# crowsonkb/k-diffusion

Measured on NVIDIA H100. Metric: images/sec (256x256, Heun 50-step), higher is better.
Workload: dtype bf16

## Files before the change

k-diffusion_b200/csrc/tc_kernels.cu:

```cuda
#include "tc_common.cuh"
#include "tc_kernels.cuh"

namespace kdb {

typedef CUresult (*EncodeTiledFn)(CUtensorMap*, CUtensorMapDataType, cuuint32_t, void*, const cuuint64_t*, const cuuint64_t*,
                                  const cuuint32_t*, const cuuint32_t*, CUtensorMapInterleave, CUtensorMapSwizzle,
                                  CUtensorMapL2promotion, CUtensorMapFloatOOBfill);

static EncodeTiledFn encode_fn() {
  static EncodeTiledFn fn = [] {
    void* p = nullptr;
    cudaDriverEntryPointQueryResult q;
    if (cudaGetDriverEntryPoint("cuTensorMapEncodeTiled", &p, cudaEnableDefault, &q) != cudaSuccess) p = nullptr;
    return reinterpret_cast<EncodeTiledFn>(p);
  }();
  return fn;
}

int make_tmap_bf16(CUtensorMap* out, const void* base, int rank, const uint64_t* dims, const uint64_t* strides_bytes, const uint32_t* box) {
  EncodeTiledFn fn = encode_fn();
  KDB_REQUIRE(fn != nullptr, KDB_ERR_UNSUPPORTED, "cuTensorMapEncodeTiled not available from this driver");
  cuuint64_t gd[5];
  cuuint64_t gs[5];
  cuuint32_t bx[5], es[5];
  for (int i = 0; i < rank; ++i) {
    gd[i] = dims[i];
    bx[i] = box[i];
    es[i] = 1;
    if (i > 0) gs[i - 1] = strides_bytes[i - 1];
  }
  CUresult r = fn(out, CU_TENSOR_MAP_DATA_TYPE_BFLOAT16, (cuuint32_t)rank, const_cast<void*>(base), gd, gs, bx, es,
                  CU_TENSOR_MAP_INTERLEAVE_NONE, CU_TENSOR_MAP_SWIZZLE_128B, CU_TENSOR_MAP_L2_PROMOTION_L2_256B,
                  CU_TENSOR_MAP_FLOAT_OOB_FILL_NONE);
  KDB_REQUIRE(r == CUDA_SUCCESS, KDB_ERR_BAD_ARG, "cuTensorMapEncodeTiled failed with CUresult %d (rank %d, dim0 %llu, box0 %u)", (int)r,
              rank, (unsigned long long)dims[0], box[0]);
  return 0;
}

int make_tmap_tokens(CUtensorMap* out, const void* base, uint64_t C, int B, int h, int w, uint32_t box_c, uint32_t box_w, uint32_t box_h) {
  const uint64_t dims[4] = {C, (uint64_t)w, (uint64_t)h, (uint64_t)B};
  const uint64_t strides[3] = {C * 2, C * 2 * w, C * 2 * w * h};
  const uint32_t box[4] = {box_c, box_w, box_h, 1};
  return make_tmap_bf16(out, base, 4, dims, strides, box);
}

bool pdl_enabled() {
  static const bool enabled = [] {
    const char* e = getenv("KDB200_NO_PDL");
    return !(e != nullptr && e[0] == '1');
  }();
  return enabled;
}

namespace {

constexpr int BM = 128, BK = 64;
constexpr int A_STAGE_BYTES = BM * BK * 2;
constexpr int SUB_TILE_BYTES = BM * 128;
constexpr int GEMM_THREADS = 384;

struct GemmArgs : GemmEpi {
  bf16* out;
  int64_t M;
  int N, K;
  int box_w, box_h;
  int th, tw;
};

__device__ __forceinline__ float bf16_round(float v) { return __bfloat162float(__float2bfloat16_rn(v)); }

int tmap_2d(CUtensorMap* t, const void* base, uint64_t inner, uint64_t outer, uint32_t box_inner, uint32_t box_outer) {
  const uint64_t dims[2] = {inner, outer};
  const uint64_t strides[1] = {inner * 2};
  const uint32_t box[2] = {box_inner, box_outer};
  return make_tmap_bf16(t, base, 2, dims, strides, box);
}

int tmap_quad(CUtensorMap* t, const void* base, int C, int wc, uint64_t bhc, int box_w, int box_h) {
  const uint64_t dims[5] = {(uint64_t)C, 2, (uint64_t)wc, 2, bhc};
  const uint64_t strides[4] = {(uint64_t)C * 2, (uint64_t)C * 4, (uint64_t)wc * C * 4, (uint64_t)wc * C * 8};
  const uint32_t box[5] = {64, 1, (uint32_t)box_w, 1, (uint32_t)box_h};
  return make_tmap_bf16(t, base, 5, dims, strides, box);
}

bool quad_box(int wc, int* box_w, int* box_h) {
  if (wc >= BM) {
    if (wc % BM != 0) return false;
    *box_w = BM;
    *box_h = 1;
    return true;
  }
  if (BM % wc != 0) return false;
  *box_w = wc;
  *box_h = BM / wc;
  return true;
}

struct QuadCoord {
  int e, nw, wx, nh, row;
};
__device__ __forceinline__ QuadCoord quad_coord(int64_t m0, int n, int C, int wc, int box_h) {
  const int qd = n / C;
  return QuadCoord{n - qd * C, qd & 1, box_h == 1 ? (int)(m0 % wc) : 0, qd >> 1, (int)(m0 / wc)};
}

template <int BN, int EPI> constexpr int out_bytes() {
  return EPI == EPI_GEGLU ? SUB_TILE_BYTES : EPI == EPI_PATCH_OUT ? 0 : (BN / 64) * SUB_TILE_BYTES;
}
template <int BN, int EPI> constexpr int acc_bytes() { return EPI == EPI_GEGLU ? 0 : BM * BN * 4; }
template <int EPI> constexpr int ring_bytes() { return EPI == EPI_GEGLU ? 192 * 1024 : 96 * 1024; }
template <int BN, int EPI> constexpr size_t gemm_smem() { return 1024 + ring_bytes<EPI>() + acc_bytes<BN, EPI>() + 2 * out_bytes<BN, EPI>() + 128; }

template <int BN> __device__ __forceinline__ int stage_off(int row, int chunk) { return row * BN + ((chunk ^ (row & 7)) << 2); }
template <int BN>
__device__ __forceinline__ void stage_store(float* s, int row0, const float (&d)[BN / 2]) {
  const int t = threadIdx.x & 127;
  const int r = row0 + 16 * (t >> 5) + ((t & 31) >> 2), c = 2 * (t & 3);
#pragma unroll
  for (int j = 0; j < BN / 8; ++j) {
    *reinterpret_cast<float2*>(s + stage_off<BN>(r, 2 * j + (c >> 2)) + (c & 3)) = make_float2(d[4 * j], d[4 * j + 1]);
    *reinterpret_cast<float2*>(s + stage_off<BN>(r + 8, 2 * j + (c >> 2)) + (c & 3)) = make_float2(d[4 * j + 2], d[4 * j + 3]);
  }
}
template <int BN>
__device__ __forceinline__ void stage_ld32(const float* s, int row, int col0, float (&v)[32]) {
#pragma unroll
  for (int i = 0; i < 8; ++i) {
    const float4 q = *reinterpret_cast<const float4*>(s + stage_off<BN>(row, (col0 >> 2) + i));
    v[4 * i] = q.x;
    v[4 * i + 1] = q.y;
    v[4 * i + 2] = q.z;
    v[4 * i + 3] = q.w;
  }
}

template <int BN, int EPI>
__global__ void __launch_bounds__(GEMM_THREADS, 1) gemm_wg_kernel(const __grid_constant__ CUtensorMap tma, const __grid_constant__ CUtensorMap tmb,
                                                                  const __grid_constant__ CUtensorMap tmc, const __grid_constant__ CUtensorMap tmr,
                                                                  const GemmArgs p) {
  KDB_PDL_TRIGGER();
  constexpr int B_STAGE_BYTES = BN * BK * 2;
  constexpr int STAGE_BYTES = A_STAGE_BYTES + B_STAGE_BYTES;
  constexpr int RING_BYTES = ring_bytes<EPI>();
  constexpr int STAGES = RING_BYTES / STAGE_BYTES;
  constexpr int NSUB = BN / 64;
  constexpr bool RES = EPI == EPI_RESID;
  uint8_t* base = tc::smem_1k();
  float* sAcc = reinterpret_cast<float*>(base + RING_BYTES);
  auto* ring = reinterpret_cast<tc::TmaRing<STAGES>*>(base + RING_BYTES + acc_bytes<BN, EPI>() + 2 * out_bytes<BN, EPI>());
  uint64_t* resid_full = reinterpret_cast<uint64_t*>(ring + 1);

  const int warp = threadIdx.x >> 5, lane = threadIdx.x & 31;
  const int nkb = p.K / BK;
  const int n_tiles = p.N / BN;
  const int n_local = tc::tiles_owned((int)((p.M + BM - 1) / BM) * n_tiles);

  if (threadIdx.x == 0) {
    tc::tma_prefetch_desc(&tma);
    tc::tma_prefetch_desc(&tmb);
    ring->init(tc::REL_WARPS);
    tc::mbar_init(&resid_full[0], 1);
    tc::mbar_init(&resid_full[1], 1);
    tc::fence_barrier_init();
  }
  __syncthreads();
  tc::pdl_wait();

  if (warp >= 8) {
    tc::setmaxnreg_dec<tc::PRODUCER_REGS>();
    if (warp == 8 && tc::elect_one()) {
      int it = 0;
      for (int i = 0; i < n_local; ++i) {
        const int t = (int)blockIdx.x + i * (int)gridDim.x;
        const int64_t m0 = (int64_t)(t / n_tiles) * BM;
        const int n0 = (t % n_tiles) * BN;
        for (int kb = 0; kb < nkb; ++kb, ++it) {
          const auto ps = PipeState<STAGES>::at(it);
          uint64_t* bar = ring->acquire(ps, STAGE_BYTES);
          uint8_t* a = base + (size_t)ps.slot * STAGE_BYTES;
          if (p.mC > 0) {
            const QuadCoord q = quad_coord(m0, kb * BK, p.mC, p.mwc, p.box_h);
            tc::tma_load_5d(a, &tma, bar, q.e, q.nw, q.wx, q.nh, q.row);
          } else {
            tc::tma_load_2d(a, &tma, bar, kb * BK, (int)m0);
          }
          tc::tma_load_2d(a + A_STAGE_BYTES, &tmb, bar, kb * BK, n0);
        }
      }
    }
    return;
  }
  tc::setmaxnreg_inc<tc::MMA_REGS>();

  const int wg = warp >> 2;
  const int row = threadIdx.x & 127;
  uint8_t* sC = base + RING_BYTES + acc_bytes<BN, EPI>() + wg * out_bytes<BN, EPI>();
  const int r0 = 16 * (warp & 3) + (lane >> 2), cq = 2 * (lane & 3);
  for (int i = wg; i < n_local; i += 2) {
    const int t = (int)blockIdx.x + i * (int)gridDim.x;
    const int64_t m0 = (int64_t)(t / n_tiles) * BM;
    const int n0 = (t % n_tiles) * BN;
    if constexpr (RES || EPI == EPI_SPLIT_LERP) {
      if (row == 0 && (RES || p.box_w > 0)) {
        tc::mbar_arrive_expect_tx(&resid_full[wg], NSUB * SUB_TILE_BYTES);
#pragma unroll
        for (int g = 0; g < NSUB; ++g) {
          if constexpr (RES) {
            tc::tma_load_2d(sC + g * SUB_TILE_BYTES, &tmr, &resid_full[wg], n0 + g * 64, (int)m0);
          } else {
            const QuadCoord q = quad_coord(m0, n0 + g * 64, p.C, p.wc, p.box_h);
            tc::tma_load_5d(sC + g * SUB_TILE_BYTES, &tmr, &resid_full[wg], q.e, q.nw, q.wx, q.nh, q.row);
          }
        }
      }
    }
    float frag_rstd[4] = {1.f, 1.f, 1.f, 1.f};
    if constexpr (EPI == EPI_GEGLU) {
      if (p.ss_in != nullptr) {
#pragma unroll
        for (int h = 0; h < 4; ++h) {
          const int64_t m = m0 + r0 + 64 * (h >> 1) + 8 * (h & 1);
          const float4* sp = reinterpret_cast<const float4*>(p.ss_in + (m < p.M ? m : 0) * SS_PARTS);
          frag_rstd[h] = rsqrtf(tc::rowss_sum(__ldg(sp), __ldg(sp + 1), p.K >> 7) / (float)p.K + 1e-6f);
        }
      }
    }

    float acc0[BN / 2], acc1[BN / 2];
#pragma unroll
    for (int k = 0; k < BN / 2; ++k) acc0[k] = acc1[k] = 0.f;
    if (i > 0) tc::named_barrier_sync(tc::BAR_TURN + wg, 256);
    const int it0 = i * nkb;
    for (int kb = 0; kb < nkb; ++kb) {
      const auto ps = PipeState<STAGES>::at(it0 + kb);
      ring->wait(ps);
      const uint32_t a_addr = tc::smem_u32(base + (size_t)ps.slot * STAGE_BYTES);
      const uint64_t ad0 = tc::smem_desc_k_sw128(a_addr), ad1 = tc::smem_desc_k_sw128(a_addr + 8 * 1024);
      const uint64_t bd = tc::smem_desc_k_sw128(a_addr + A_STAGE_BYTES);
      tc::wg_fence_acc(acc0);
      tc::wg_fence_acc(acc1);
      tc::wg_fence();
#pragma unroll
      for (int k = 0; k < BK / 16; ++k) {
        if constexpr (BN == 128) {
          tc::wgmma_128(acc0, ad0 + 2ull * k, bd + 2ull * k, 1u);
          tc::wgmma_128(acc1, ad1 + 2ull * k, bd + 2ull * k, 1u);
        } else {
          tc::wgmma_64<0>(acc0, ad0 + 2ull * k, bd + 2ull * k, 1u);
          tc::wgmma_64<0>(acc1, ad1 + 2ull * k, bd + 2ull * k, 1u);
        }
      }
      tc::wg_commit();
      tc::wg_wait<1>();
      tc::wg_fence_acc(acc0);
      tc::wg_fence_acc(acc1);
      if (kb > 0 && lane == 0) ring->release(PipeState<STAGES>::at(it0 + kb - 1));
    }
    if (i + 1 < n_local) tc::named_barrier_arrive(tc::BAR_TURN + (wg ^ 1), 256);
    tc::wg_wait<0>();
    tc::wg_fence_acc(acc0);
    tc::wg_fence_acc(acc1);
    if (lane == 0) ring->release(PipeState<STAGES>::at(it0 + nkb - 1));

    if constexpr (EPI == EPI_GEGLU) {
      tc::named_barrier_sync(tc::BAR_WG + wg, 128);
#pragma unroll
      for (int half = 0; half < 2; ++half) {
        const float r_a = frag_rstd[2 * half], r_b = frag_rstd[2 * half + 1];
        uint32_t o[16];
        tc::geglu_fragment(half == 0 ? acc0 : acc1, tc::pk2(0.5f * r_a, 0.5f * r_a), tc::pk2(0.5f * r_b, 0.5f * r_b), tc::pk2(r_a, r_a),
                           tc::pk2(r_b, r_b), o);
        const int r = 64 * half + r0;
#pragma unroll
        for (int q = 0; q < 8; ++q) {
          *reinterpret_cast<uint32_t*>(sC + tc::sw128_offset(r, q) + 2 * cq) = o[2 * q];
          *reinterpret_cast<uint32_t*>(sC + tc::sw128_offset(r + 8, q) + 2 * cq) = o[2 * q + 1];
        }
      }
      tc::fence_proxy_async();
      tc::named_barrier_sync(tc::BAR_WG + wg, 128);
      if (row == 0) {
        tc::tma_store_2d(&tmc, sC, n0 / 2, (int)m0);
        tc::tma_store_commit();
        tc::tma_store_wait_read();
      }
      continue;
    }
    if (i > 0) tc::named_barrier_sync(tc::BAR_ACC + wg, 256);
    stage_store<BN>(sAcc, 0, acc0);
    stage_store<BN>(sAcc, 64, acc1);
    tc::named_barrier_sync(tc::BAR_WG + wg, 128);
    const bool pass_acc = i + 1 < n_local;

    const int64_t m = m0 + row;
    float rstd = 1.f;
    if (p.ss_in != nullptr) {
      const float4* sp = reinterpret_cast<const float4*>(p.ss_in + (m < p.M ? m : 0) * SS_PARTS);
      rstd = rsqrtf(tc::rowss_sum(__ldg(sp), __ldg(sp + 1), p.K >> 7) / (float)p.K + 1e-6f);
    }
    if constexpr (EPI == EPI_PATCH_OUT) {
      float v[64];
      {
        float t0[32], t1[32];
        stage_ld32<BN>(sAcc, row, 0, t0);
        stage_ld32<BN>(sAcc, row, 32, t1);
#pragma unroll
        for (int k = 0; k < 32; ++k) { v[k] = t0[k]; v[32 + k] = t1[k]; }
      }
      if (pass_acc) tc::named_barrier_arrive(tc::BAR_ACC + (wg ^ 1), 256);
      if (m < p.M) {
        if (p.ss_in != nullptr) {
#pragma unroll
          for (int k = 0; k < 48; ++k) v[k] *= rstd;
        }
        const int per = p.th * p.tw;
        const int b = (int)(m / per);
        const int r = (int)(m - (int64_t)b * per);
        const int ty = r / p.tw, tx = r - ty * p.tw;
        float c_skip = 0.f, c_out = 1.f, c_in;
        if (p.sigma_data > 0.f) karras_scalings(__ldg(p.sigma + b), p.sigma_data, c_skip, c_out, c_in);
#pragma unroll
        for (int c = 0; c < 3; ++c)
#pragma unroll
          for (int nh = 0; nh < 4; ++nh) {
            const int64_t o = (((int64_t)b * 3 + c) * p.H + (ty * 4 + nh)) * p.W + tx * 4;
            float4 y = make_float4(bf16_round(v[(nh * 4 + 0) * 3 + c]), bf16_round(v[(nh * 4 + 1) * 3 + c]), bf16_round(v[(nh * 4 + 2) * 3 + c]),
                                   bf16_round(v[(nh * 4 + 3) * 3 + c]));
            if (p.sigma_data > 0.f) {
              const float4 xi = __ldg(reinterpret_cast<const float4*>(p.x_in + o));
              y = make_float4(y.x * c_out + xi.x * c_skip, y.y * c_out + xi.y * c_skip, y.z * c_out + xi.z * c_skip, y.w * c_out + xi.w * c_skip);
            }
            *reinterpret_cast<float4*>(p.img + o) = y;
          }
      }
    } else if constexpr (EPI == EPI_SPLIT_LERP) {
      const bool live = m < p.M;
      const float facv = __ldg(p.fac);
      float ss = 0.f;
      int64_t fine = 0;
      if (p.box_w > 0) {
        tc::mbar_wait_nocall(&resid_full[wg], (uint32_t)(i >> 1) & 1u);
#pragma unroll 1
        for (int g = 0; g < NSUB; ++g) {
          float v[64];
          {
            float t0[32], t1[32];
            stage_ld32<BN>(sAcc, row, g * 64, t0);
            stage_ld32<BN>(sAcc, row, g * 64 + 32, t1);
#pragma unroll
            for (int k = 0; k < 32; ++k) { v[k] = t0[k]; v[32 + k] = t1[k]; }
          }
          if (g == NSUB - 1 && pass_acc) tc::named_barrier_arrive(tc::BAR_ACC + (wg ^ 1), 256);
          uint8_t* cg = sC + g * SUB_TILE_BYTES;
#pragma unroll
          for (int j = 0; j < 8; ++j) {
            uint4* cp = reinterpret_cast<uint4*>(cg + tc::sw128_offset(row, j));
            const uint4 r4 = *cp;
            const uint32_t rw[4] = {r4.x, r4.y, r4.z, r4.w};
            uint32_t ow[4];
#pragma unroll
            for (int q = 0; q < 4; ++q) {
              const float lo = __uint_as_float(rw[q] << 16), hi = __uint_as_float(rw[q] & 0xffff0000u);
              const float e0 = v[j * 8 + q * 2], e1 = v[j * 8 + q * 2 + 1];
              const float d0 = e0 - lo, d1 = e1 - hi;
              const float o0 = (facv < 0.5f) ? fmaf(facv, d0, lo) : e0 - d0 * (1.f - facv);
              const float o1 = (facv < 0.5f) ? fmaf(facv, d1, hi) : e1 - d1 * (1.f - facv);
              ss = fmaf(o0, o0, fmaf(o1, o1, ss));
              ow[q] = tc::pack_bf16x2(o0, o1);
            }
            *cp = make_uint4(ow[0], ow[1], ow[2], ow[3]);
          }
        }
        if (p.ss_out != nullptr && live) {
          const int64_t b = m / ((int64_t)p.hc * p.wc);
          const int r = (int)(m - b * p.hc * p.wc);
          const int hy = r / p.wc, wx = r - hy * p.wc, qd = n0 / p.C;
          fine = (b * (2 * p.hc) + (2 * hy + (qd >> 1))) * (2 * p.wc) + (2 * wx + (qd & 1));
          p.ss_out[fine * SS_PARTS + ((n0 % p.C) >> 7)] = ss;
        }
        tc::fence_proxy_async();
        tc::named_barrier_sync(tc::BAR_WG + wg, 128);
        if (row == 0) {
#pragma unroll
          for (int g = 0; g < NSUB; ++g) {
            const QuadCoord q = quad_coord(m0, n0 + g * 64, p.C, p.wc, p.box_h);
            tc::tma_store_5d(&tmc, sC + g * SUB_TILE_BYTES, q.e, q.nw, q.wx, q.nh, q.row);
          }
          tc::tma_store_commit();
          tc::tma_store_wait_read();
        }
        continue;
      }
#pragma unroll 1
      for (int c = 0; c < BN / 32; ++c) {
        float v[32];
        stage_ld32<BN>(sAcc, row, c * 32, v);
        if (c == BN / 32 - 1 && pass_acc) tc::named_barrier_arrive(tc::BAR_ACC + (wg ^ 1), 256);
        if (!live) continue;
        const int n = n0 + c * 32;
        const int64_t b = m / ((int64_t)p.hc * p.wc);
        const int r = (int)(m - b * p.hc * p.wc);
        const int hy = r / p.wc, wx = r - hy * p.wc;
        const int qd = n / p.C, e = n - qd * p.C;
        fine = (b * (2 * p.hc) + (2 * hy + (qd >> 1))) * (2 * p.wc) + (2 * wx + (qd & 1));
        const int64_t off = fine * p.C + e;
        const uint4* sk = reinterpret_cast<const uint4*>(static_cast<const bf16*>(p.resid) + off);
        uint4* dst = reinterpret_cast<uint4*>(p.out + off);
#pragma unroll
        for (int j = 0; j < 4; ++j) {
          const uint4 r4 = sk[j];
          const uint32_t rw[4] = {r4.x, r4.y, r4.z, r4.w};
          uint32_t ow[4];
#pragma unroll
          for (int q = 0; q < 4; ++q) {
            const float lo = __uint_as_float(rw[q] << 16), hi = __uint_as_float(rw[q] & 0xffff0000u);
            const float e0 = v[j * 8 + q * 2], e1 = v[j * 8 + q * 2 + 1];
            const float d0 = e0 - lo, d1 = e1 - hi;
            const float o0 = (facv < 0.5f) ? fmaf(facv, d0, lo) : e0 - d0 * (1.f - facv);
            const float o1 = (facv < 0.5f) ? fmaf(facv, d1, hi) : e1 - d1 * (1.f - facv);
            ss = fmaf(o0, o0, fmaf(o1, o1, ss));
            ow[q] = tc::pack_bf16x2(o0, o1);
          }
          dst[j] = make_uint4(ow[0], ow[1], ow[2], ow[3]);
        }
      }
      if (p.ss_out != nullptr && live) p.ss_out[fine * SS_PARTS + ((n0 % p.C) >> 7)] = ss;
    } else {
      if constexpr (RES) tc::mbar_wait_nocall(&resid_full[wg], (uint32_t)(i >> 1) & 1u);
      float ss_acc[4] = {0.f, 0.f, 0.f, 0.f};
#pragma unroll 1
      for (int g = 0; g < NSUB; ++g) {
        float v[64];
        {
          float t0[32], t1[32];
          stage_ld32<BN>(sAcc, row, g * 64, t0);
          stage_ld32<BN>(sAcc, row, g * 64 + 32, t1);
#pragma unroll
          for (int k = 0; k < 32; ++k) { v[k] = t0[k]; v[32 + k] = t1[k]; }
        }
        if (g == NSUB - 1 && pass_acc) tc::named_barrier_arrive(tc::BAR_ACC + (wg ^ 1), 256);
        if (p.ss_in != nullptr) {
          bool apply = true;
          if constexpr (EPI == EPI_QKV_ROPE) apply = (n0 + g * 64) >= 2 * p.C;
          if (apply) {
#pragma unroll
            for (int k = 0; k < 64; ++k) v[k] *= rstd;
          }
        }
        uint8_t* cg = sC + g * SUB_TILE_BYTES;
        if constexpr (RES) {
#pragma unroll
          for (int j = 0; j < 8; ++j) {
            const uint4 r4 = *reinterpret_cast<const uint4*>(cg + tc::sw128_offset(row, j));
            const uint32_t rw[4] = {r4.x, r4.y, r4.z, r4.w};
#pragma unroll
            for (int q = 0; q < 4; ++q) {
              v[j * 8 + q * 2] += __uint_as_float(rw[q] << 16);
              v[j * 8 + q * 2 + 1] += __uint_as_float(rw[q] & 0xffff0000u);
            }
          }
        }
        if constexpr (RES || EPI == EPI_STORE) {
          if (p.ss_out != nullptr) {
#pragma unroll
            for (int k = 0; k < 64; k += 4) {
              ss_acc[0] = fmaf(v[k], v[k], ss_acc[0]);
              ss_acc[1] = fmaf(v[k + 1], v[k + 1], ss_acc[1]);
              ss_acc[2] = fmaf(v[k + 2], v[k + 2], ss_acc[2]);
              ss_acc[3] = fmaf(v[k + 3], v[k + 3], ss_acc[3]);
            }
          }
        }
        if constexpr (EPI == EPI_QKV_ROPE) {
          const int n = n0 + g * 64;
          const int t3 = n / p.C, head = (n - t3 * p.C) >> 6;
          if (t3 < 2) {
            const int64_t tok = (m < p.M ? m : 0) % p.T_tokens;
            const float4* tb = reinterpret_cast<const float4*>(p.rope) + (int64_t)head * 8 * p.T_tokens + tok;
            tc::f32x2 P[32];
#pragma unroll
            for (int k = 0; k < 32; ++k) P[k] = tc::pk2(v[2 * k], v[2 * k + 1]);
            tc::f32x2 q0 = tc::mul2(P[0], P[0]), q1 = tc::mul2(P[1], P[1]), q2 = tc::mul2(P[2], P[2]), q3 = tc::mul2(P[3], P[3]);
#pragma unroll
            for (int k = 4; k < 32; k += 4) {
              q0 = tc::fma2(P[k], P[k], q0);
              q1 = tc::fma2(P[k + 1], P[k + 1], q1);
              q2 = tc::fma2(P[k + 2], P[k + 2], q2);
              q3 = tc::fma2(P[k + 3], P[k + 3], q3);
            }
            const float sc = sqrtf(__ldg(p.qk_scale + head)) * rsqrtf(((q0.x + q0.y) + (q1.x + q1.y)) + ((q2.x + q2.y) + (q3.x + q3.y)) + 1e-6f);
            const tc::f32x2 sc2 = tc::pk2(sc, sc);
#pragma unroll
            for (int k = 0; k < 8; ++k) {
              const float4 cs = __ldg(tb + (int64_t)k * p.T_tokens);
              const tc::f32x2 C = tc::pk2(cs.x, cs.y), S = tc::pk2(cs.z, cs.w);
              const tc::f32x2 X1 = P[k], X2 = P[8 + k];
              P[k] = tc::mul2(tc::fma2(X2, tc::neg2(S), tc::mul2(X1, C)), sc2);
              P[8 + k] = tc::mul2(tc::fma2(X1, S, tc::mul2(X2, C)), sc2);
            }
#pragma unroll
            for (int k = 16; k < 32; ++k) P[k] = tc::mul2(P[k], sc2);
#pragma unroll
            for (int k = 0; k < 32; ++k) tc::upk2(P[k], v[2 * k], v[2 * k + 1]);
          }
        }
#pragma unroll
        for (int j = 0; j < 8; ++j)
          *reinterpret_cast<uint4*>(cg + tc::sw128_offset(row, j)) =
              make_uint4(tc::pack_bf16x2(v[j * 8 + 0], v[j * 8 + 1]), tc::pack_bf16x2(v[j * 8 + 2], v[j * 8 + 3]),
                         tc::pack_bf16x2(v[j * 8 + 4], v[j * 8 + 5]), tc::pack_bf16x2(v[j * 8 + 6], v[j * 8 + 7]));
      }
      if constexpr (RES || EPI == EPI_STORE) {
        if (p.ss_out != nullptr && m < p.M) p.ss_out[m * SS_PARTS + (n0 >> 7)] = (ss_acc[0] + ss_acc[1]) + (ss_acc[2] + ss_acc[3]);
      }
      tc::fence_proxy_async();
      tc::named_barrier_sync(tc::BAR_WG + wg, 128);
      if (row == 0) {
#pragma unroll
        for (int g = 0; g < NSUB; ++g) tc::tma_store_2d(&tmc, sC + g * SUB_TILE_BYTES, n0 + g * 64, (int)m0);
        tc::tma_store_commit();
        tc::tma_store_wait_read();
      }
    }
  }
}


#include "tc_ffn_fused.cuh"
#include "tc_attn_block.cuh"

template <int BN, int EPI>
int launch_tc(const bf16* A, const bf16* W, const GemmArgs& p, cudaStream_t st) {
  CUtensorMap ta, tb, tcm, tr;
  int rc;
  if (p.mC > 0) {
    if ((rc = tmap_quad(&ta, A, p.mC, p.mwc, (uint64_t)p.M / p.mwc, p.box_w, p.box_h))) return rc;
  } else {
    if ((rc = tmap_2d(&ta, A, (uint64_t)p.K, (uint64_t)p.M, BK, BM))) return rc;
  }
  if ((rc = tmap_2d(&tb, W, (uint64_t)p.K, (uint64_t)p.N, BK, BN))) return rc;
  const uint64_t n_out = EPI == EPI_GEGLU ? (uint64_t)p.N / 2 : (uint64_t)p.N;
  if (EPI == EPI_SPLIT_LERP && p.box_w > 0) {
    if ((rc = tmap_quad(&tcm, p.out, p.C, p.wc, (uint64_t)p.M / p.wc, p.box_w, p.box_h))) return rc;
    if ((rc = tmap_quad(&tr, p.resid, p.C, p.wc, (uint64_t)p.M / p.wc, p.box_w, p.box_h))) return rc;
  } else {
    if (EPI != EPI_SPLIT_LERP && EPI != EPI_PATCH_OUT) {
      if ((rc = tmap_2d(&tcm, p.out, n_out, (uint64_t)p.M, 64, BM))) return rc;
    } else {
      tcm = ta;
    }
    if (EPI == EPI_RESID) {
      if ((rc = tmap_2d(&tr, p.resid, (uint64_t)p.N, (uint64_t)p.M, 64, BM))) return rc;
    } else {
      tr = ta;
    }
  }
  constexpr size_t smem = gemm_smem<BN, EPI>();
  static_assert(smem <= 227 * 1024, "GEMM shared memory exceeds the 227 KiB opt-in limit");
  static bool opened = false;
  if ((rc = set_smem_once(gemm_wg_kernel<BN, EPI>, opened, (int)smem))) return rc;
  KDB_CUDA(launch_pdl(gemm_wg_kernel<BN, EPI>, persistent_grid(ceil_div(p.M, BM) * (p.N / BN)), dim3(GEMM_THREADS), smem, st, ta, tb, tcm, tr, p));
  KDB_LAUNCH_CHECK(EPI == EPI_PATCH_OUT ? F_PATCH_OUT : F_GEMM_TC, st);
  return 0;
}

template <int EPI>
int dispatch_bn(const bf16* A, const bf16* W, const GemmArgs& p, cudaStream_t st) {
  if (p.N % 128 == 0) return launch_tc<128, EPI>(A, W, p, st);
  return launch_tc<64, EPI>(A, W, p, st);
}

bool shape_ok(int64_t M, int N, int K) {
  return M > 0 && M < (65535LL * BM) && N >= 64 && N % 64 == 0 && K >= 64 && K % 64 == 0;
}

bool aligned16(const void* p) { return (reinterpret_cast<uintptr_t>(p) & 15) == 0; }

bool rowss_fits(int N, const GemmEpi& epi) {
  if (N % 128 != 0) return false;
  if (epi.mode == EPI_RESID || epi.mode == EPI_STORE) return N <= 128 * SS_PARTS;
  if (epi.mode == EPI_SPLIT_LERP) return epi.C % 128 == 0 && epi.C <= 128 * SS_PARTS;
  return false;
}

bool gemm_fits(int64_t M, int N, int K, const GemmEpi& epi) {
  if (!shape_ok(M, N, K)) return false;
  if (epi.ss_in != nullptr) {
    if (K % 128 != 0 || K > 128 * SS_PARTS || epi.mC > 0 || epi.mode == EPI_RESID || epi.mode == EPI_SPLIT_LERP) return false;
    if ((epi.mode == EPI_STORE || epi.mode == EPI_QKV_ROPE) && N % 128 != 0) return false;
  }
  if (epi.ss_out != nullptr && !rowss_fits(N, epi)) return false;
  if (epi.mC > 0) {
    int bw, bh;
    if (epi.mode != EPI_STORE || N % 128 != 0 || epi.mC % 64 != 0 || K != 4 * epi.mC || M % epi.mwc != 0 || !quad_box(epi.mwc, &bw, &bh)) return false;
  }
  switch (epi.mode) {
    case EPI_STORE:
    case EPI_RESID:
      return true;
    case EPI_GEGLU:
      return N % 128 == 0;
    case EPI_SPLIT_LERP:
      return epi.C % 32 == 0 && N == 4 * epi.C;
    case EPI_QKV_ROPE:
      return N == 3 * epi.C && epi.C % 64 == 0 && epi.nh * 64 == epi.C && epi.rope != nullptr;
    case EPI_PATCH_OUT:
      return N == 64 && epi.W % 4 == 0 && aligned16(epi.img) && (epi.sigma_data <= 0.f || aligned16(epi.x_in));
    default:
      return false;
  }
}

}

namespace {
struct PatchInParams {
  const float* x;
  const float* sigma;
  float sd;
  int64_t M;
  int H, Wimg, th, tw, N;
  float* ss_out;
};

constexpr int PATCH_IN_THREADS = 160;
constexpr int PATCH_IN_LD = 132;
constexpr size_t PATCH_IN_SMEM = 1024 + 2 * A_STAGE_BYTES + (size_t)BM * PATCH_IN_LD * 4 + 2 * SUB_TILE_BYTES + 64;

__global__ void __launch_bounds__(PATCH_IN_THREADS) patch_in_tc_kernel(const __grid_constant__ CUtensorMap tmw, const __grid_constant__ CUtensorMap tmc,
                                                                   const PatchInParams p) {
  KDB_PDL_TRIGGER();
  constexpr int LD = PATCH_IN_LD;
  uint8_t* sA = tc::smem_1k();
  uint8_t* sW = sA + A_STAGE_BYTES;
  uint8_t* sC = sW + A_STAGE_BYTES;
  float* sAcc = reinterpret_cast<float*>(sC + 2 * SUB_TILE_BYTES);
  uint64_t* w_full = reinterpret_cast<uint64_t*>(sAcc + BM * LD);

  const int warp = threadIdx.x >> 5;
  const int64_t m0 = (int64_t)blockIdx.x * BM;
  const int n0 = blockIdx.y * 128;
  if (threadIdx.x == 0) {
    tc::tma_prefetch_desc(&tmw);
    tc::tma_prefetch_desc(&tmc);
    tc::mbar_init(w_full, 1);
    tc::fence_barrier_init();
  }
  __syncthreads();

  if (warp == 4) {
    if (tc::elect_one()) {
      tc::mbar_arrive_expect_tx(w_full, A_STAGE_BYTES);
      tc::tma_load_2d(sW, &tmw, w_full, 0, n0);
    }
    return;
  }
  const int row = threadIdx.x;
  const int64_t m = m0 + row;
  uint4 chunk[6];
  if (m < p.M) {
    const int per = p.th * p.tw;
    const int b = (int)(m / per);
    const int r = (int)(m - (int64_t)b * per);
    const int ty = r / p.tw, tx = r - ty * p.tw;
    float c_in = 1.f;
    if (p.sd > 0.f) {
      const float sg = __ldg(p.sigma + b);
      c_in = rsqrtf(fmaf(sg, sg, p.sd * p.sd));
    }
    float4 px[12];
#pragma unroll
    for (int c = 0; c < 3; ++c)
#pragma unroll
      for (int nh = 0; nh < 4; ++nh)
        px[c * 4 + nh] = __ldg(reinterpret_cast<const float4*>(p.x + (((int64_t)b * 3 + c) * p.H + (ty * 4 + nh)) * p.Wimg + tx * 4));
#pragma unroll
    for (int j = 0; j < 6; ++j) {
      const float4 a = px[2 * j], bq = px[2 * j + 1];
      chunk[j] = make_uint4(tc::pack_bf16x2(a.x * c_in, a.y * c_in), tc::pack_bf16x2(a.z * c_in, a.w * c_in), tc::pack_bf16x2(bq.x * c_in, bq.y * c_in),
                            tc::pack_bf16x2(bq.z * c_in, bq.w * c_in));
    }
  } else {
#pragma unroll
    for (int j = 0; j < 6; ++j) chunk[j] = make_uint4(0u, 0u, 0u, 0u);
  }
#pragma unroll
  for (int j = 0; j < 6; ++j) *reinterpret_cast<uint4*>(sA + tc::sw128_offset(row, j)) = chunk[j];
  *reinterpret_cast<uint4*>(sA + tc::sw128_offset(row, 6)) = make_uint4(0u, 0u, 0u, 0u);
  *reinterpret_cast<uint4*>(sA + tc::sw128_offset(row, 7)) = make_uint4(0u, 0u, 0u, 0u);
  tc::fence_proxy_async();
  tc::named_barrier_sync(1, 128);
  tc::mbar_wait_nocall(w_full, 0);
  {
    float acc0[64], acc1[64];
    const uint32_t a_addr = tc::smem_u32(sA);
    const uint64_t ad0 = tc::smem_desc_k_sw128(a_addr), ad1 = tc::smem_desc_k_sw128(a_addr + 8 * 1024), bd = tc::smem_desc_k_sw128(tc::smem_u32(sW));
#pragma unroll
    for (int i = 0; i < 64; ++i) acc0[i] = acc1[i] = 0.f;
    tc::wg_fence_acc(acc0);
    tc::wg_fence_acc(acc1);
    tc::wg_fence();
#pragma unroll
    for (int k = 0; k < BK / 16; ++k) {
      tc::wgmma_128(acc0, ad0 + 2ull * k, bd + 2ull * k, 1u);
      tc::wgmma_128(acc1, ad1 + 2ull * k, bd + 2ull * k, 1u);
    }
    tc::wg_commit();
    tc::wg_wait<0>();
    tc::wg_fence_acc(acc0);
    tc::wg_fence_acc(acc1);
    tc::acc_store(sAcc, LD, 0, acc0);
    tc::acc_store(sAcc, LD, 64, acc1);
  }
  tc::named_barrier_sync(1, 128);
  float ss0 = 0.f, ss1 = 0.f;
#pragma unroll
  for (int g = 0; g < 2; ++g) {
    float v[64];
    {
      float t0[32], t1[32];
      tc::acc_ld32(sAcc, LD, row, g * 64, t0);
      tc::acc_ld32(sAcc, LD, row, g * 64 + 32, t1);
#pragma unroll
      for (int i = 0; i < 32; ++i) { v[i] = t0[i]; v[32 + i] = t1[i]; }
    }
#pragma unroll
    for (int i = 0; i < 64; i += 2) {
      ss0 = fmaf(v[i], v[i], ss0);
      ss1 = fmaf(v[i + 1], v[i + 1], ss1);
    }
    uint8_t* cg = sC + g * SUB_TILE_BYTES;
#pragma unroll
    for (int j = 0; j < 8; ++j)
      *reinterpret_cast<uint4*>(cg + tc::sw128_offset(row, j)) =
          make_uint4(tc::pack_bf16x2(v[j * 8 + 0], v[j * 8 + 1]), tc::pack_bf16x2(v[j * 8 + 2], v[j * 8 + 3]),
                     tc::pack_bf16x2(v[j * 8 + 4], v[j * 8 + 5]), tc::pack_bf16x2(v[j * 8 + 6], v[j * 8 + 7]));
  }
  if (p.ss_out != nullptr && m < p.M) p.ss_out[m * SS_PARTS + (n0 >> 7)] = ss0 + ss1;
  tc::fence_proxy_async();
  tc::named_barrier_sync(1, 128);
  if (threadIdx.x == 0) {
    tc::tma_store_2d(&tmc, sC, n0, (int)m0);
    tc::tma_store_2d(&tmc, sC + SUB_TILE_BYTES, n0 + 64, (int)m0);
    tc::tma_store_commit();
    tc::tma_store_wait_read();
  }
}

__global__ void __launch_bounds__(256) patch_in_weight_kernel(const float* __restrict__ W, bf16* __restrict__ out, int N) {
  for (int i = blockIdx.x * 256 + threadIdx.x; i < N * 64; i += gridDim.x * 256) {
    const int n = i >> 6, k = i & 63;
    float v = 0.f;
    if (k < 48) {
      const int c = k >> 4, nh = (k >> 2) & 3, nw = k & 3;
      v = W[(int64_t)n * 48 + (nh * 4 + nw) * 3 + c];
    }
    out[i] = __float2bfloat16(v);
  }
}

}

static bool g_tc_disabled = [] {
  const char* e = getenv("KDB200_DISABLE_TC");
  return e != nullptr && e[0] == '1';
}();

bool tc_gemm_supported(int64_t M, int N, int K, const GemmEpi& epi) { return !g_tc_disabled && gemm_fits(M, N, K, epi); }

bool tc_gemm_emits_rowss(int64_t M, int N, int K, const GemmEpi& epi) { return tc_gemm_supported(M, N, K, epi) && rowss_fits(N, epi); }

int launch_gemm_tc(const bf16* A, const bf16* W, bf16* C, int64_t M, int N, int K, const GemmEpi& epi, cudaStream_t st) {
  KDB_REQUIRE(aligned16(A) && aligned16(W) && aligned16(C), KDB_ERR_BAD_ARG, "gemm_tc: operands must be 16-byte aligned");
  KDB_REQUIRE(gemm_fits(M, N, K, epi), KDB_ERR_UNSUPPORTED, "gemm_tc: epilogue %d does not support M=%lld N=%d K=%d with these options", epi.mode,
              (long long)M, N, K);
  GemmArgs p{};
  static_cast<GemmEpi&>(p) = epi;
  p.out = C;
  p.M = M;
  p.N = N;
  p.K = K;
  p.th = epi.H / 4;
  p.tw = epi.W / 4;
  if (epi.mC > 0) {
    quad_box(epi.mwc, &p.box_w, &p.box_h);
    return launch_tc<128, EPI_STORE>(A, W, p, st);
  }
  if (epi.mode == EPI_SPLIT_LERP && epi.C % 64 == 0 && epi.wc > 0 && M % epi.wc == 0 && aligned16(epi.resid)) quad_box(epi.wc, &p.box_w, &p.box_h);
  switch (epi.mode) {
    case EPI_STORE:
      return dispatch_bn<EPI_STORE>(A, W, p, st);
    case EPI_RESID:
      return dispatch_bn<EPI_RESID>(A, W, p, st);
    case EPI_GEGLU:
      return launch_tc<128, EPI_GEGLU>(A, W, p, st);
    case EPI_SPLIT_LERP:
      return dispatch_bn<EPI_SPLIT_LERP>(A, W, p, st);
    case EPI_QKV_ROPE:
      return dispatch_bn<EPI_QKV_ROPE>(A, W, p, st);
    case EPI_PATCH_OUT:
      return launch_tc<64, EPI_PATCH_OUT>(A, W, p, st);
    default:
      return KDB_ERR_BAD_ARG;
  }
}

bool tc_patch_in_supported(const float* x, int C0, int Wimg) {
  return !g_tc_disabled && C0 % 128 == 0 && C0 <= 128 * SS_PARTS && Wimg % 4 == 0 && aligned16(x);
}

int prepare_patch_in_weight(const float* W, bf16* out, int C0, cudaStream_t st) {
  patch_in_weight_kernel<<<(unsigned)ceil_div((int64_t)C0 * 64, 256), 256, 0, st>>>(W, out, C0);
  KDB_LAUNCH_CHECK(F_CONVERT, st);
  return 0;
}

int launch_patch_in_tc(const float* x, const float* sigma, float sigma_data, const bf16* W_perm, bf16* out, int B, int H, int Wimg, int C0,
                       float* ss_out, cudaStream_t st) {
  PatchInParams p{};
  p.x = x;
  p.sigma = sigma;
  p.sd = sigma_data;
  p.H = H;
  p.Wimg = Wimg;
  p.th = H / 4;
  p.tw = Wimg / 4;
  p.M = (int64_t)B * p.th * p.tw;
  p.N = C0;
  p.ss_out = ss_out;
  KDB_REQUIRE(tc_patch_in_supported(x, C0, Wimg), KDB_ERR_UNSUPPORTED,
              "patch_in_tc: needs C0 %% 128 == 0, C0 <= %d, W %% 4 == 0 and a 16-byte aligned input (got C0=%d W=%d)", 128 * SS_PARTS, C0, Wimg);
  CUtensorMap tw, tcm;
  int rc;
  if ((rc = tmap_2d(&tw, W_perm, 64, (uint64_t)C0, 64, 128))) return rc;
  if ((rc = tmap_2d(&tcm, out, (uint64_t)C0, (uint64_t)p.M, 64, BM))) return rc;
  static bool opened = false;
  if ((rc = set_smem_once(patch_in_tc_kernel, opened, (int)PATCH_IN_SMEM))) return rc;
  patch_in_tc_kernel<<<dim3((unsigned)ceil_div(p.M, BM), (unsigned)(C0 / 128)), PATCH_IN_THREADS, PATCH_IN_SMEM, st>>>(tw, tcm, p);
  KDB_LAUNCH_CHECK(F_PATCH_IN, st);
  return 0;
}

__global__ void __launch_bounds__(256) fold_norm_weights_kernel(const FoldDesc* __restrict__ descs, const float* __restrict__ cond) {
  KDB_PDL_TRIGGER();
  const FoldDesc d = descs[blockIdx.y];
  const int64_t chunks = (int64_t)d.rows * d.K / 8;
  const float* g = cond + d.ada_off;
  for (int64_t i = (int64_t)blockIdx.x * 256 + threadIdx.x; i < chunks; i += (int64_t)gridDim.x * 256) {
    const int k0 = (int)((i * 8) % d.K);
    const uint4 raw = __ldg(reinterpret_cast<const uint4*>(d.src) + i);
    const uint32_t w[4] = {raw.x, raw.y, raw.z, raw.w};
    uint32_t o[4];
#pragma unroll
    for (int t = 0; t < 4; ++t) {
      const float lo = __uint_as_float(w[t] << 16) * __ldg(g + k0 + 2 * t), hi = __uint_as_float(w[t] & 0xffff0000u) * __ldg(g + k0 + 2 * t + 1);
      o[t] = tc::pack_bf16x2(lo, hi);
    }
    reinterpret_cast<uint4*>(d.dst)[i] = make_uint4(o[0], o[1], o[2], o[3]);
  }
}

int launch_fold_norm_weights(const FoldDesc* descs_dev, int n_desc, const float* cond_row, cudaStream_t st) {
  if (n_desc <= 0) return 0;
  fold_norm_weights_kernel<<<dim3(48, (unsigned)n_desc), 256, 0, st>>>(descs_dev, cond_row);
  KDB_LAUNCH_CHECK(F_FUSED_NORM, st);
  return 0;
}

bool tc_ffn_fused_supported(int64_t M, int C, int dff) {
  static const bool off = [] {
    const char* e = getenv("KDB200_NO_FFN_FUSE");
    return e != nullptr && e[0] == '1';
  }();
  return !off && !g_tc_disabled && ffn_fused_supported(M, C, dff);
}

int launch_ffn_fused(bf16* x, const bf16* w_up_il, const bf16* w_down, int64_t M, int C, int dff, const float* ss_in, float* ss_out, cudaStream_t st) {
  KDB_REQUIRE(ffn_fused_supported(M, C, dff) && ss_in != nullptr, KDB_ERR_BAD_SHAPE, "ffn_fused: unsupported shape (needs C = 128, M %% 128 == 0, d_ff %% 64 == 0)");
  return launch_ffn_fused_impl(x, w_up_il, w_down, M, dff, ss_in, ss_out, st);
}

bool tc_attn_block_supported(int h, int w, int C, int nh, int e, int attn_type, int attn_param, int shift) {
  return !g_tc_disabled && attn_block_supported(h, w, C, nh, e, attn_type, attn_param, shift);
}

int launch_attn_block(bf16* x, const bf16* w_qkv, const bf16* w_out, const float2* rope, const float* qk_scale, int B, int h, int w, int shift,
                      const float* ss_in, float* ss_out, cudaStream_t st) {
  KDB_REQUIRE(B > 0 && attn_block_supported(h, w, AB_C, 2, 64, KDB_ATTN_SHIFTED_WINDOW, 8, shift), KDB_ERR_BAD_SHAPE,
              "attn_block: unsupported shape (needs C = 128, two heads of 64, window 8, shift 0 or 4, h %% 8 == 0, w %% 8 == 0; got B=%d h=%d w=%d shift=%d)",
              B, h, w, shift);
  return launch_attn_block_impl(x, w_qkv, w_out, rope, qk_scale, B, h, w, shift, ss_in, ss_out, st);
}

}

extern "C" int kdb_gemm_bf16(const void* a, const void* w, void* c, int M, int N, int K, void* stream) {
  using namespace kdb;
  KDB_REQUIRE(a && w && c, KDB_ERR_BAD_ARG, "gemm_bf16: NULL operand");
  GemmEpi e;
  KDB_REQUIRE(shape_ok(M, N, K), KDB_ERR_UNSUPPORTED, "gemm_bf16: needs N %% 64 == 0 and K %% 64 == 0 (got M=%d N=%d K=%d)", M, N, K);
  return launch_gemm_tc(static_cast<const bf16*>(a), static_cast<const bf16*>(w), static_cast<bf16*>(c), M, N, K, e, (cudaStream_t)stream);
}

extern "C" int kdb_gemm_bf16_geglu(const void* a, const void* w_il, void* c, int M, int N2, int K, const float* ss_in, void* stream) {
  using namespace kdb;
  KDB_REQUIRE(a && w_il && c, KDB_ERR_BAD_ARG, "gemm_bf16_geglu: NULL operand");
  GemmEpi e;
  e.mode = EPI_GEGLU;
  e.ss_in = ss_in;
  KDB_REQUIRE(tc_gemm_supported(M, N2, K, e), KDB_ERR_UNSUPPORTED,
              "gemm_bf16_geglu: needs N2 %% 128 == 0 and K %% 64 == 0 (K %% 128 == 0, K <= 1024 with ss_in); got M=%d N2=%d K=%d", M, N2, K);
  return launch_gemm_tc(static_cast<const bf16*>(a), static_cast<const bf16*>(w_il), static_cast<bf16*>(c), M, N2, K, e, (cudaStream_t)stream);
}

extern "C" int kdb_ffn_fused_bf16(void* x, const void* w_up_il, const void* w_down, int M, int d_ff, const float* ss_in, float* ss_out, void* stream) {
  using namespace kdb;
  KDB_REQUIRE(x && w_up_il && w_down && ss_in, KDB_ERR_BAD_ARG, "ffn_fused_bf16: NULL operand");
  return launch_ffn_fused(static_cast<bf16*>(x), static_cast<const bf16*>(w_up_il), static_cast<const bf16*>(w_down), M, 128, d_ff, ss_in, ss_out,
                          (cudaStream_t)stream);
}

extern "C" int kdb_attn_block_bf16(void* x, const void* w_qkv, const void* w_out, const float* rope, const float* qk_scale, int batch, int h, int w,
                                   int shift, const float* ss_in, float* ss_out, void* stream) {
  using namespace kdb;
  KDB_REQUIRE(x && w_qkv && w_out && rope && qk_scale && ss_in && ss_out, KDB_ERR_BAD_ARG, "attn_block_bf16: NULL operand");
  return launch_attn_block(static_cast<bf16*>(x), static_cast<const bf16*>(w_qkv), static_cast<const bf16*>(w_out), reinterpret_cast<const float2*>(rope),
                           qk_scale, batch, h, w, shift, ss_in, ss_out, (cudaStream_t)stream);
}
```

Baseline: 132.0.

## Keep A tile resident in smem across grouped N tiles for GEGLU GEMM

Adds a resident-A variant of the warp-specialized GEMM for the GEGLU epilogue. When K is small, the whole A row-block stays in shared memory and a group of consecutive N tiles is computed against it, so only W streams through the ring. A host heuristic picks the group size so the persistent-grid wave count does not grow. It also moves TMA store read-waits to just before the staging buffer is reused, letting stores overlap with the next tile. The cost is more complex barrier bookkeeping and fewer W stages when A is resident.

```diff
diff --git a/k-diffusion_b200/csrc/tc_kernels.cu b/k-diffusion_b200/csrc/tc_kernels.cu
--- a/k-diffusion_b200/csrc/tc_kernels.cu
+++ b/k-diffusion_b200/csrc/tc_kernels.cu
@@ -65,6 +65,7 @@
   int N, K;
   int box_w, box_h;
   int th, tw;
+  int g;
 };
 
 __device__ __forceinline__ float bf16_round(float v) { return __bfloat162float(__float2bfloat16_rn(v)); }
@@ -109,7 +110,11 @@
 }
 template <int BN, int EPI> constexpr int acc_bytes() { return EPI == EPI_GEGLU ? 0 : BM * BN * 4; }
 template <int EPI> constexpr int ring_bytes() { return EPI == EPI_GEGLU ? 192 * 1024 : 96 * 1024; }
-template <int BN, int EPI> constexpr size_t gemm_smem() { return 1024 + ring_bytes<EPI>() + acc_bytes<BN, EPI>() + 2 * out_bytes<BN, EPI>() + 128; }
+constexpr int GEMM_BAR_BYTES = 512;
+template <int BN, int EPI> constexpr size_t gemm_smem() {
+  return 1024 + ring_bytes<EPI>() + acc_bytes<BN, EPI>() + 2 * out_bytes<BN, EPI>() + GEMM_BAR_BYTES;
+}
+constexpr int RESIDENT_SLOTS = 4;
 
 template <int BN> __device__ __forceinline__ int stage_off(int row, int chunk) { return row * BN + ((chunk ^ (row & 7)) << 2); }
 template <int BN>
@@ -134,31 +139,43 @@
   }
 }
 
-template <int BN, int EPI>
-__global__ void __launch_bounds__(GEMM_THREADS, 1) gemm_wg_kernel(const __grid_constant__ CUtensorMap tma, const __grid_constant__ CUtensorMap tmb,
-                                                                  const __grid_constant__ CUtensorMap tmc, const __grid_constant__ CUtensorMap tmr,
-                                                                  const GemmArgs p) {
+template <int BN, int EPI, int ACAP>
+__device__ __forceinline__ void gemm_wg(const CUtensorMap& tma, const CUtensorMap& tmb, const CUtensorMap& tmc, const CUtensorMap& tmr,
+                                        const GemmArgs& p) {
   KDB_PDL_TRIGGER();
   constexpr int B_STAGE_BYTES = BN * BK * 2;
-  constexpr int STAGE_BYTES = A_STAGE_BYTES + B_STAGE_BYTES;
+  constexpr int STAGE_BYTES = (ACAP > 0 ? 0 : A_STAGE_BYTES) + B_STAGE_BYTES;
   constexpr int RING_BYTES = ring_bytes<EPI>();
-  constexpr int STAGES = RING_BYTES / STAGE_BYTES;
+  constexpr int STAGES = (RING_BYTES - ACAP * A_STAGE_BYTES) / STAGE_BYTES;
   constexpr int NSUB = BN / 64;
   constexpr bool RES = EPI == EPI_RESID;
+  constexpr int ASLOTS = ACAP > 0 ? ACAP : 1;
+  using ARing = tc::TmaRing<ASLOTS>;
+  static_assert(ACAP == 0 || (BN == 128 && STAGES >= 2), "the resident-A walk runs 128-wide tiles with at least two W stages");
+  static_assert(sizeof(tc::TmaRing<STAGES>) + (ACAP > 0 ? sizeof(ARing) : 0) + 2 * sizeof(uint64_t) <= GEMM_BAR_BYTES, "GEMM barriers");
   uint8_t* base = tc::smem_1k();
+  uint8_t* stages = base + ACAP * A_STAGE_BYTES;
   float* sAcc = reinterpret_cast<float*>(base + RING_BYTES);
   auto* ring = reinterpret_cast<tc::TmaRing<STAGES>*>(base + RING_BYTES + acc_bytes<BN, EPI>() + 2 * out_bytes<BN, EPI>());
-  uint64_t* resid_full = reinterpret_cast<uint64_t*>(ring + 1);
+  auto* aring = reinterpret_cast<ARing*>(ring + 1);
+  uint64_t* resid_full = reinterpret_cast<uint64_t*>(ACAP > 0 ? reinterpret_cast<uint8_t*>(aring + 1) : reinterpret_cast<uint8_t*>(ring + 1));
 
   const int warp = threadIdx.x >> 5, lane = threadIdx.x & 31;
   const int nkb = p.K / BK;
-  const int n_tiles = p.N / BN;
-  const int n_local = tc::tiles_owned((int)((p.M + BM - 1) / BM) * n_tiles);
+  const int per_item = ACAP > 0 ? p.g : 1;
+  const int groups = p.N / BN / per_item;
+  const int n_local = tc::tiles_owned((int)((p.M + BM - 1) / BM) * groups) * per_item;
+  auto tile_origin = [&](int j, int tq, int64_t& m0, int& n0) {
+    const int u = (int)blockIdx.x + j * (int)gridDim.x;
+    m0 = (int64_t)(u / groups) * BM;
+    n0 = ((u % groups) * per_item + tq) * BN;
+  };
 
   if (threadIdx.x == 0) {
     tc::tma_prefetch_desc(&tma);
     tc::tma_prefetch_desc(&tmb);
     ring->init(tc::REL_WARPS);
+    if constexpr (ACAP > 0) aring->init(tc::REL_WARPS_2WG);
     tc::mbar_init(&resid_full[0], 1);
     tc::mbar_init(&resid_full[1], 1);
     tc::fence_barrier_init();
@@ -171,20 +188,30 @@
     if (warp == 8 && tc::elect_one()) {
       int it = 0;
       for (int i = 0; i < n_local; ++i) {
-        const int t = (int)blockIdx.x + i * (int)gridDim.x;
-        const int64_t m0 = (int64_t)(t / n_tiles) * BM;
-        const int n0 = (t % n_tiles) * BN;
+        const int j = i / per_item, tq = i - j * per_item;
+        int64_t m0;
+        int n0;
+        tile_origin(j, tq, m0, n0);
         for (int kb = 0; kb < nkb; ++kb, ++it) {
           const auto ps = PipeState<STAGES>::at(it);
-          uint64_t* bar = ring->acquire(ps, STAGE_BYTES);
-          uint8_t* a = base + (size_t)ps.slot * STAGE_BYTES;
-          if (p.mC > 0) {
-            const QuadCoord q = quad_coord(m0, kb * BK, p.mC, p.mwc, p.box_h);
-            tc::tma_load_5d(a, &tma, bar, q.e, q.nw, q.wx, q.nh, q.row);
+          if constexpr (ACAP > 0) {
+            if (tq == 0) {
+              uint64_t* abar = aring->acquire(PipeState<ASLOTS>::at(j * ASLOTS + kb), A_STAGE_BYTES);
+              tc::tma_load_2d(base + (size_t)kb * A_STAGE_BYTES, &tma, abar, kb * BK, (int)m0);
+            }
+            uint64_t* bar = ring->acquire(ps, STAGE_BYTES);
+            tc::tma_load_2d(stages + (size_t)ps.slot * STAGE_BYTES, &tmb, bar, kb * BK, n0);
           } else {
-            tc::tma_load_2d(a, &tma, bar, kb * BK, (int)m0);
+            uint64_t* bar = ring->acquire(ps, STAGE_BYTES);
+            uint8_t* a = base + (size_t)ps.slot * STAGE_BYTES;
+            if (p.mC > 0) {
+              const QuadCoord qc = quad_coord(m0, kb * BK, p.mC, p.mwc, p.box_h);
+              tc::tma_load_5d(a, &tma, bar, qc.e, qc.nw, qc.wx, qc.nh, qc.row);
+            } else {
+              tc::tma_load_2d(a, &tma, bar, kb * BK, (int)m0);
+            }
+            tc::tma_load_2d(a + A_STAGE_BYTES, &tmb, bar, kb * BK, n0);
           }
-          tc::tma_load_2d(a + A_STAGE_BYTES, &tmb, bar, kb * BK, n0);
         }
       }
     }
@@ -197,11 +224,14 @@
   uint8_t* sC = base + RING_BYTES + acc_bytes<BN, EPI>() + wg * out_bytes<BN, EPI>();
   const int r0 = 16 * (warp & 3) + (lane >> 2), cq = 2 * (lane & 3);
   for (int i = wg; i < n_local; i += 2) {
-    const int t = (int)blockIdx.x + i * (int)gridDim.x;
-    const int64_t m0 = (int64_t)(t / n_tiles) * BM;
-    const int n0 = (t % n_tiles) * BN;
+    const int j = i / per_item, tq = i - j * per_item;
+    const bool release_a = ACAP > 0 && tq + 2 >= per_item;
+    int64_t m0;
+    int n0;
+    tile_origin(j, tq, m0, n0);
     if constexpr (RES || EPI == EPI_SPLIT_LERP) {
       if (row == 0 && (RES || p.box_w > 0)) {
+        tc::tma_store_wait_read();
         tc::mbar_arrive_expect_tx(&resid_full[wg], NSUB * SUB_TILE_BYTES);
 #pragma unroll
         for (int g = 0; g < NSUB; ++g) {
@@ -234,9 +264,17 @@
     for (int kb = 0; kb < nkb; ++kb) {
       const auto ps = PipeState<STAGES>::at(it0 + kb);
       ring->wait(ps);
-      const uint32_t a_addr = tc::smem_u32(base + (size_t)ps.slot * STAGE_BYTES);
+      uint32_t a_addr, b_addr;
+      if constexpr (ACAP > 0) {
+        aring->wait(PipeState<ASLOTS>::at(j * ASLOTS + kb));
+        a_addr = tc::smem_u32(base + (size_t)kb * A_STAGE_BYTES);
+        b_addr = tc::smem_u32(stages + (size_t)ps.slot * STAGE_BYTES);
+      } else {
+        a_addr = tc::smem_u32(base + (size_t)ps.slot * STAGE_BYTES);
+        b_addr = a_addr + A_STAGE_BYTES;
+      }
       const uint64_t ad0 = tc::smem_desc_k_sw128(a_addr), ad1 = tc::smem_desc_k_sw128(a_addr + 8 * 1024);
-      const uint64_t bd = tc::smem_desc_k_sw128(a_addr + A_STAGE_BYTES);
+      const uint64_t bd = tc::smem_desc_k_sw128(b_addr);
       tc::wg_fence_acc(acc0);
       tc::wg_fence_acc(acc1);
       tc::wg_fence();
@@ -254,15 +292,22 @@
       tc::wg_wait<1>();
       tc::wg_fence_acc(acc0);
       tc::wg_fence_acc(acc1);
-      if (kb > 0 && lane == 0) ring->release(PipeState<STAGES>::at(it0 + kb - 1));
+      if (kb > 0 && lane == 0) {
+        ring->release(PipeState<STAGES>::at(it0 + kb - 1));
+        if (release_a) aring->release(PipeState<ASLOTS>::at(j * ASLOTS + kb - 1));
+      }
     }
     if (i + 1 < n_local) tc::named_barrier_arrive(tc::BAR_TURN + (wg ^ 1), 256);
     tc::wg_wait<0>();
     tc::wg_fence_acc(acc0);
     tc::wg_fence_acc(acc1);
-    if (lane == 0) ring->release(PipeState<STAGES>::at(it0 + nkb - 1));
+    if (lane == 0) {
+      ring->release(PipeState<STAGES>::at(it0 + nkb - 1));
+      if (release_a) aring->release(PipeState<ASLOTS>::at(j * ASLOTS + nkb - 1));
+    }
 
     if constexpr (EPI == EPI_GEGLU) {
+      if (row == 0) tc::tma_store_wait_read();
       tc::named_barrier_sync(tc::BAR_WG + wg, 128);
 #pragma unroll
       for (int half = 0; half < 2; ++half) {
@@ -282,13 +327,13 @@
       if (row == 0) {
         tc::tma_store_2d(&tmc, sC, n0 / 2, (int)m0);
         tc::tma_store_commit();
-        tc::tma_store_wait_read();
       }
       continue;
     }
     if (i > 0) tc::named_barrier_sync(tc::BAR_ACC + wg, 256);
     stage_store<BN>(sAcc, 0, acc0);
     stage_store<BN>(sAcc, 64, acc1);
+    if (row == 0) tc::tma_store_wait_read();
     tc::named_barrier_sync(tc::BAR_WG + wg, 128);
     const bool pass_acc = i + 1 < n_local;
 
@@ -387,7 +432,6 @@
             tc::tma_store_5d(&tmc, sC + g * SUB_TILE_BYTES, q.e, q.nw, q.wx, q.nh, q.row);
           }
           tc::tma_store_commit();
-          tc::tma_store_wait_read();
         }
         continue;
       }
@@ -519,17 +563,30 @@
 #pragma unroll
         for (int g = 0; g < NSUB; ++g) tc::tma_store_2d(&tmc, sC + g * SUB_TILE_BYTES, n0 + g * 64, (int)m0);
         tc::tma_store_commit();
-        tc::tma_store_wait_read();
-      }
-    }
-  }
+      }
+    }
+  }
+  if (row == 0) tc::tma_store_wait_read();
+}
+
+template <int BN, int EPI>
+__global__ void __launch_bounds__(GEMM_THREADS, 1) gemm_wg_kernel(const __grid_constant__ CUtensorMap tma, const __grid_constant__ CUtensorMap tmb,
+                                                                  const __grid_constant__ CUtensorMap tmc, const __grid_constant__ CUtensorMap tmr,
+                                                                  const __grid_constant__ GemmArgs p) {
+  gemm_wg<BN, EPI, 0>(tma, tmb, tmc, tmr, p);
+}
+template <int EPI, int ACAP>
+__global__ void __launch_bounds__(GEMM_THREADS, 1)
+    gemm_wg_resident_kernel(const __grid_constant__ CUtensorMap tma, const __grid_constant__ CUtensorMap tmb, const __grid_constant__ CUtensorMap tmc,
+                            const __grid_constant__ CUtensorMap tmr, const __grid_constant__ GemmArgs p) {
+  gemm_wg<128, EPI, ACAP>(tma, tmb, tmc, tmr, p);
 }
 
 
 #include "tc_ffn_fused.cuh"
 #include "tc_attn_block.cuh"
 
-template <int BN, int EPI>
+template <int BN, int EPI, int ACAP = 0>
 int launch_tc(const bf16* A, const bf16* W, const GemmArgs& p, cudaStream_t st) {
   CUtensorMap ta, tb, tcm, tr;
   int rc;
@@ -557,11 +614,37 @@
   }
   constexpr size_t smem = gemm_smem<BN, EPI>();
   static_assert(smem <= 227 * 1024, "GEMM shared memory exceeds the 227 KiB opt-in limit");
+  auto* kernel = gemm_wg_kernel<BN, EPI>;
+  if constexpr (ACAP > 0) kernel = gemm_wg_resident_kernel<EPI, ACAP>;
+  const int64_t items = ceil_div(p.M, BM) * (p.N / BN) / (ACAP > 0 ? p.g : 1);
   static bool opened = false;
-  if ((rc = set_smem_once(gemm_wg_kernel<BN, EPI>, opened, (int)smem))) return rc;
-  KDB_CUDA(launch_pdl(gemm_wg_kernel<BN, EPI>, persistent_grid(ceil_div(p.M, BM) * (p.N / BN)), dim3(GEMM_THREADS), smem, st, ta, tb, tcm, tr, p));
+  if ((rc = set_smem_once(kernel, opened, (int)smem))) return rc;
+  KDB_CUDA(launch_pdl(kernel, persistent_grid(items), dim3(GEMM_THREADS), smem, st, ta, tb, tcm, tr, p));
   KDB_LAUNCH_CHECK(EPI == EPI_PATCH_OUT ? F_PATCH_OUT : F_GEMM_TC, st);
   return 0;
+}
+
+int resident_group(int64_t M, int n_tiles) {
+  const int64_t blocks = ceil_div(M, BM), sms = num_sms();
+  int best = 1;
+  int64_t best_span = ceil_div(blocks * n_tiles, sms);
+  for (int g = 2; g <= n_tiles; ++g) {
+    if (n_tiles % g != 0) continue;
+    const int64_t span = ceil_div(blocks * (n_tiles / g), sms) * g;
+    if (span <= best_span) {
+      best = g;
+      best_span = span;
+    }
+  }
+  return best;
+}
+
+int launch_geglu(const bf16* A, const bf16* W, GemmArgs p, cudaStream_t st) {
+  p.g = p.K <= 2 * RESIDENT_SLOTS * BK ? resident_group(p.M, p.N / 128) : 1;
+  if (p.K <= RESIDENT_SLOTS * BK && p.g > 1) return launch_tc<128, EPI_GEGLU, RESIDENT_SLOTS>(A, W, p, st);
+  if (p.K > RESIDENT_SLOTS * BK && p.g >= 4) return launch_tc<128, EPI_GEGLU, 2 * RESIDENT_SLOTS>(A, W, p, st);
+  p.g = 1;
+  return launch_tc<128, EPI_GEGLU>(A, W, p, st);
 }
 
 template <int EPI>
@@ -793,7 +876,7 @@
     case EPI_RESID:
       return dispatch_bn<EPI_RESID>(A, W, p, st);
     case EPI_GEGLU:
-      return launch_tc<128, EPI_GEGLU>(A, W, p, st);
+      return launch_geglu(A, W, p, st);
     case EPI_SPLIT_LERP:
       return dispatch_bn<EPI_SPLIT_LERP>(A, W, p, st);
     case EPI_QKV_ROPE:
```

After: 134.1 (median of 6 runs). +1.6%, better.
